# OpenGene/gencore

Hardware: AMD Instinct MI355X
Metric: consensus read-pairs/sec (whole node) + clustering HBM GB/s vs roofline (higher is better)
Workload: dtype u8

## Files before the change

gencore_amd/csrc/engine.hip:

```cpp
#include <hip/hip_runtime.h>
#include <hip/hip_ext.h>
#include <cstdio>
#include <cstdlib>
#include <algorithm>
#include <cstring>
#include <ctime>
#include <string>
#include <vector>

#include "gce_entry.h"
#include "gce_kernels.hpp"
#include "gce_params.hpp"
#include "gce_pair2.hpp"
#include "gce_vote.hpp"
#include "gce_deep.hpp"
#include "gce_output.hpp"
#include "gce_depth.hpp"
#include "gce_inflate.hpp"
#include "gce_deflate.hpp"

namespace {

static thread_local double t_alloc_s = 0.0; static thread_local long t_alloc_n = 0; static thread_local size_t t_alloc_bytes = 0;
static inline double mono_s() { struct timespec ts; clock_gettime(CLOCK_MONOTONIC, &ts); return (double)ts.tv_sec + 1e-9 * (double)ts.tv_nsec; }
// ... 22 lines not shown
struct ScopedBuf : DevBuf { ~ScopedBuf() { release(); } };
template <class T> inline hipError_t ensure_as(DevBuf &d, T *&dst, size_t bytes) { const hipError_t r = d.ensure(bytes); dst = d.as<T>(); return r; }

enum { EV_START = 0, EV_CLUSTER, EV_CSR, EV_DESCRIBE, EV_PAIRING, EV_SCORE, EV_CONSENSUS, EV_FINISH, EV_OUTPUT, EV_COUNT };

}

#include "gce_devstream.hpp"

struct HostRaw {
    uint8_t *p = nullptr; size_t n = 0, cap = 0;
    ~HostRaw() { free(p); }
    void resize(size_t k) { if (k > cap) { free(p); p = (uint8_t *)malloc(k ? k : 1); cap = p ? k : 0; } n = p ? k : 0; }
    uint8_t *data() { return p; }
    size_t size() const { return n; }
    bool empty() const { return n == 0; }
};

struct gce_engine {
    gce_params prm{};
    bool vote_off_logged = false;
    std::vector<uint32_t> target_len;
    std::string err;
    hipStream_t stream = nullptr;
    hipEvent_t ev[EV_COUNT]{};
    std::vector<DevBuf> ref_buf; std::vector<const uint8_t *> ref_ptr; std::vector<int64_t> ref_len, ref_win; bool have_win = false;
    DevBuf d_ref_ptr, d_ref_len, d_ref_win, d_target_len, d_target_cum;
    std::vector<const uint8_t *> up_ref_ptr; std::vector<int64_t> up_ref_len, up_win; std::vector<uint32_t> up_tl; const void *up_dev[5]{}; bool up_valid = false;
    std::vector<gce_core> h_core; std::vector<uint64_t> h_qoff, h_coff, h_soff, h_loff, h_mioff;
    std::vector<char> h_qname, h_mi; std::vector<uint32_t> h_cigar; std::vector<uint8_t> h_seq, h_qual, h_nmt; std::vector<int32_t> h_nm; std::vector<uint64_t> h_tick;
    std::vector<int32_t> h_ev_tid, h_ev_pos;
    bool have_mi = false, have_tick = false, have_events = false, host_mode = false, device_mode = false, processed = false;
    bool reserved = false; hipStream_t up_stream = nullptr; std::vector<hipEvent_t> up_events;
    hipStream_t aux_stream = nullptr; hipEvent_t aux_ev[4]{};
    size_t rs_n = 0, rs_q = 0, rs_c = 0, rs_s = 0, rs_l = 0, st_n = 0, st_q = 0, st_c = 0, st_s = 0, st_l = 0, st_m = 0; bool dev_concat = false;
    gce_batch dev_batch{};
    DevBuf b_core, b_qoff, b_qname, b_coff, b_cigar, b_soff, b_seq, b_loff, b_qual, b_nm, b_nmt, b_mioff, b_mi, b_tick;
    DevBuf uinfo, rdesc, spatch, slot, score, out_flag, orec, out_index, nmx;
    DevBuf o_src, o_kind, o_qsrc, o_nm, o_fr, o_rr, o_mate, o_soff, o_qoff, o_seq, o_qual, o_key, o_rec, o_ksoff, o_kqoff, o_krow, o_rank64, o_part3, ref_ascii;
    int64_t n_out = 0; size_t out_seq_bytes = 0, out_qual_bytes = 0; int dev_error = 0; uint32_t dev_error_read = 0;
    DevBuf lrec, lout, bhdr, blk_base, ev_tid, ev_pos, ev_read, table, toff;
    DevBuf raw, rw_tmp, rw_ncig, rw_nmpos, rw_rsize, rw_roff, rw_body; RecIdx rw;
    size_t raw_n = 0; bool raw_mode = false; int64_t raw_records = 0; uint64_t raw_body_bytes = 0;
    int64_t idx_ctr[4] = {0, 0, 0, 0};
    DevBuf z_comp, z_dir, z_err; size_t z_n = 0; std::vector<InfDir> z_members;
    DevBuf zo_slots, zo_sizes, zo_off, zo_out; uint64_t zo_bytes = 0;
    DevBuf sf_text; uint64_t sf_bytes = 0; int64_t raw_body_nrec = -1;
    std::vector<gce_engine *> mirrors;
    DevBuf sh_tickall, sh_shard, sh_flag, sh_sel, sh_core, sh_qoff, sh_coff, sh_soff, sh_loff, sh_nm, sh_nmt, sh_mioff, sh_tick, sh_roff, sh_nmpos, sh_keys, sh_stage; int64_t shard_n = -1;
    bool shard_cut_done = false;
    bool tab_clean = false; const void *tab_clean_ptr = nullptr; size_t tab_clean_cap = 0;
    DevBuf cl_ikey, cl_start, cl_n, cl_npairs, cl_ngroups, cl_gbase, cl_nresult, cl_hasumi, cl_tier;
    DevBuf members, sorted, pl, pr, pu, pg, gpl, gpr, grp_begin, grp_n, gl_cluster, g_begin, g_np;
    DevBuf slow_args, deep_list, k64, slow_list, left_list, pf_flag, pf_list, pq_flag, pq_list, p16_flag, p16_list, pd_slab, gen_flag, gen_list, score_list, gw, vlive, vb_start, rp_left, rp_right, rp_merge, rp_rmerge, rp_umi, rp_umilen, rp_state, rp_supp, rp_nm, rp_qsl, rp_qsr, scan_part, si;
    StreamInfo h_si{};
    void *si_pin = nullptr, *si_pin_dev = nullptr; unsigned long long si_seq = 0;
    gce_timing timing{};
    int64_t n = 0, n_pre = 0;
    DevBuf dp_binoff, dp_regoff, dp_rs, dp_re, dp_pmax, dp_sorted, dp_depth, dp_bed, dp_where;
    std::vector<int64_t> h_binoff, h_depth_pre, h_depth_post, h_bed_pre, h_bed_post; int64_t payload_words = 0;
    std::vector<uint8_t> r_kind; HostRaw r_seq, r_qual; std::vector<uint32_t> r_src, r_qsrc, r_mate; std::vector<int32_t> r_nm; std::vector<int16_t> r_fr, r_rr;
    std::vector<uint64_t> r_soff, r_qoff;
};

static int fail(gce_engine *e, int code, const std::string &msg) { if (e) e->err = msg; return code; }
#define HIPCHK(call) do { hipError_t _e = (call); if (_e != hipSuccess) return fail(e, _e == hipErrorOutOfMemory ? GCE_ERR_OOM : GCE_ERR_HIP, std::string(#call) + ": " + hipGetErrorString(_e)); } while (0)

extern "C" {

int gce_abi_version(void) { return GCE_ABI_VERSION; }

void gce_params_default(gce_params *p) {
    memset(p, 0, sizeof *p);
    p->abi_version = GCE_ABI_VERSION;
    p->proper_umi_diff_threshold = 1; p->unproper_umi_diff_threshold = 0; p->duplex_mismatch_threshold = 2;
    p->cluster_size_req = 1; p->base_score_req = 6; p->high_quality = 30; p->moderate_quality = 20; p->low_quality = 15;
    p->score_high = 8; p->score_moderate = 6; p->score_low = 4; p->score_bad = 2;
    p->skip_low_complexity_cluster_threshold = 1000; p->flush_period = 10000; p->score_percent_req = 0.8;
}

void gce_detect_umi_prefix(const char *q, char out[32]) {
    memset(out, 0, 32);
    if (strstr(q, "umi_")) strcpy(out, "umi");
    else if (strstr(q, "UMI_")) strcpy(out, "UMI");
}

const char *gce_status_message(int s) {
    switch (s) {
    case GCE_OK: return "ok";
    case GCE_ERR_INVALID: return "invalid argument or call order";
    case GCE_ERR_NO_DEVICE: return "no HIP device available (this engine has no CPU fallback)";
    case GCE_ERR_HIP: return "HIP runtime error";
    case GCE_ERR_OOM: return "out of device memory";
    case GCE_ERR_UNSORTED: return "ERROR: the input is unsorted. Please sort the input first.";
    case GCE_ERR_UMI_MISMATCH: return "The UMI of a read pair should be identical";
    case GCE_ERR_NM_MISSING: return "NM tag missing on a consensus template whose mismatch count changed";
    case GCE_ERR_UMI_PARSE: return "UMI parse: substr start beyond the end of the read name";
    case GCE_ERR_QNAME_SHORT: return "copyQName ERROR: desitination qname is shorter";
    case GCE_ERR_REF_WINDOW: return "reference window: a clustered read lies outside the bases staged for its contig";
    default: return "unknown status";
    }
}

const char *gce_last_error(const gce_engine *e) { return e ? e->err.c_str() : "null engine"; }

int gce_create(const gce_params *params, gce_engine **out) {
    if (!params || !out || params->abi_version != GCE_ABI_VERSION) return GCE_ERR_INVALID;
    if (params->proper_umi_diff_threshold < 0 || params->unproper_umi_diff_threshold < 0 || params->flush_period < 0) return GCE_ERR_INVALID;
    int ndev = 0;
    if (hipGetDeviceCount(&ndev) != hipSuccess || ndev <= 0 || params->device >= ndev) return GCE_ERR_NO_DEVICE;
    gce_engine *e = new gce_engine();
    e->prm = *params;
    if (e->prm.flush_period == 0) e->prm.flush_period = 10000;
    if (params->n_targets > 0 && params->target_len) e->target_len.assign(params->target_len, params->target_len + params->n_targets);
    e->prm.target_len = nullptr;
    if (hipSetDevice(params->device) != hipSuccess || hipStreamCreate(&e->stream) != hipSuccess) { delete e; return GCE_ERR_HIP; }
    for (auto &v : e->ev) (void)hipEventCreate(&v);
    *out = e;
    return GCE_OK;
}

void gce_destroy(gce_engine *e) {
    if (!e) return;
    (void)hipSetDevice(e->prm.device);
    (void)hipStreamSynchronize(e->stream);
    DevBuf *all[] = {&e->d_ref_ptr, &e->d_ref_len, &e->d_ref_win, &e->d_target_len, &e->d_target_cum, &e->b_core, &e->b_qoff, &e->b_qname, &e->b_coff, &e->b_cigar, &e->b_soff,
                     &e->b_seq, &e->b_loff, &e->b_qual, &e->b_nm, &e->b_nmt, &e->b_mioff, &e->b_mi, &e->b_tick, &e->uinfo, &e->rdesc, &e->spatch,
                     &e->slot, &e->score, &e->out_flag, &e->orec, &e->out_index, &e->nmx, &e->o_src, &e->o_kind, &e->o_qsrc, &e->o_nm, &e->o_fr, &e->o_rr, &e->o_mate,
                     &e->o_key, &e->o_rec, &e->o_ksoff, &e->o_kqoff, &e->o_krow, &e->o_rank64, &e->o_part3, &e->o_soff, &e->o_qoff, &e->o_seq, &e->o_qual, &e->ref_ascii, &e->lrec, &e->lout, &e->bhdr,
                     &e->blk_base, &e->ev_tid, &e->ev_pos, &e->ev_read, &e->table, &e->toff, &e->cl_ikey, &e->cl_start, &e->cl_n,
                     &e->cl_npairs, &e->cl_ngroups, &e->cl_gbase, &e->cl_nresult, &e->cl_hasumi, &e->cl_tier, &e->members, &e->sorted, &e->pl, &e->pr, &e->pu,
                     &e->pg, &e->gpl, &e->gpr, &e->grp_begin, &e->grp_n, &e->gl_cluster, &e->g_begin, &e->g_np, &e->deep_list, &e->k64, &e->slow_list, &e->pf_flag, &e->pf_list, &e->pq_flag, &e->pq_list, &e->left_list, &e->slow_args, &e->pd_slab, &e->gen_flag, &e->gen_list, &e->score_list, &e->gw, &e->vlive, &e->vb_start, &e->rp_left, &e->rp_right, &e->rp_merge, &e->rp_rmerge,
                     &e->rp_umi, &e->rp_umilen, &e->rp_state, &e->rp_supp, &e->rp_nm, &e->rp_qsl, &e->rp_qsr, &e->scan_part, &e->si};
    for (auto *b : all) b->release();
    for (DevBuf *b : {&e->z_comp, &e->z_dir, &e->z_err, &e->raw, &e->rw_tmp, &e->rw_ncig, &e->rw_nmpos, &e->rw_rsize, &e->rw_roff, &e->rw_body, &e->sf_text}) b->release();
    e->rw.release();
    for (DevBuf *b : {&e->zo_slots, &e->zo_sizes, &e->zo_off, &e->zo_out, &e->p16_flag, &e->p16_list}) b->release();
    for (DevBuf *b : {&e->sh_tickall, &e->sh_shard, &e->sh_flag, &e->sh_sel, &e->sh_core, &e->sh_qoff, &e->sh_coff, &e->sh_soff, &e->sh_loff, &e->sh_nm, &e->sh_nmt, &e->sh_mioff, &e->sh_tick, &e->sh_roff, &e->sh_nmpos, &e->sh_keys, &e->sh_stage}) b->release();
    for (DevBuf *b : {&e->dp_binoff, &e->dp_regoff, &e->dp_rs, &e->dp_re, &e->dp_pmax, &e->dp_sorted, &e->dp_depth, &e->dp_bed, &e->dp_where}) b->release();
    for (auto ev : e->up_events) (void)hipEventDestroy(ev);
    if (e->up_stream) { (void)hipStreamSynchronize(e->up_stream); (void)hipStreamDestroy(e->up_stream); }
    if (e->aux_stream) { (void)hipStreamSynchronize(e->aux_stream); (void)hipStreamDestroy(e->aux_stream); }
    for (auto &v : e->aux_ev) if (v) (void)hipEventDestroy(v);
    for (auto &b : e->ref_buf) b.release();
    for (auto &v : e->ev) if (v) (void)hipEventDestroy(v);
    if (e->stream) (void)hipStreamDestroy(e->stream);
    if (e->si_pin) (void)hipHostFree(e->si_pin);
    delete e;
}

void gce_pack_reference(const char *bases, int64_t n, uint8_t *out) {
    memset(out, 0, (size_t)((n + 1) / 2));
    for (int64_t i = 0; i < n; i++) {
        uint8_t code;
        switch (bases[i]) { case 'A': code = 1; break; case 'T': code = 2; break; case 'C': code = 3; break; case 'G': code = 4; break; default: code = 0; }
        out[i >> 1] |= (i & 1) ? (uint8_t)(code << 4) : code;
    }
}

int gce_set_reference(gce_engine *e, int32_t tid, const uint8_t *nibbles, int64_t n_bases) {
    if (!e || tid < 0 || n_bases < 0) return GCE_ERR_INVALID;
    (void)hipSetDevice(e->prm.device);
    if ((size_t)tid >= e->ref_buf.size()) { e->ref_buf.resize(tid + 1); e->ref_ptr.resize(tid + 1, nullptr); e->ref_len.resize(tid + 1, 0); }
    if (!nibbles) { e->ref_ptr[tid] = nullptr; e->ref_len[tid] = 0; return GCE_OK; }
    size_t bytes = (size_t)((n_bases + 1) / 2);
    HIPCHK(e->ref_buf[tid].ensure(bytes + 16));
    hipPointerAttribute_t attr; bool is_dev = hipPointerGetAttributes(&attr, nibbles) == hipSuccess && attr.type == hipMemoryTypeDevice;
    (void)hipGetLastError();
    HIPCHK(hipMemcpyAsync(e->ref_buf[tid].p, nibbles, bytes, is_dev ? hipMemcpyDeviceToDevice : hipMemcpyHostToDevice, e->stream));
    HIPCHK(hipStreamSynchronize(e->stream));
    e->ref_ptr[tid] = e->ref_buf[tid].as<uint8_t>(); e->ref_len[tid] = n_bases;
    if (2 * (size_t)tid + 1 < e->ref_win.size()) e->ref_win[2 * tid] = e->ref_win[2 * tid + 1] = 0;
    return GCE_OK;
}

int gce_set_reference_ascii(gce_engine *e, int32_t tid, const char *bases, int64_t n_bases) {
    if (!e || tid < 0 || n_bases < 0 || (!bases && n_bases > 0)) return GCE_ERR_INVALID;
    (void)hipSetDevice(e->prm.device);
    if ((size_t)tid >= e->ref_buf.size()) { e->ref_buf.resize(tid + 1); e->ref_ptr.resize(tid + 1, nullptr); e->ref_len.resize(tid + 1, 0); }
    const size_t bytes = (size_t)((n_bases + 1) / 2);
    HIPCHK(e->ref_buf[tid].ensure(bytes + 16));
    HIPCHK(e->ref_ascii.ensure((size_t)n_bases + 16));
    hipPointerAttribute_t attr; const bool is_dev = hipPointerGetAttributes(&attr, bases) == hipSuccess && attr.type == hipMemoryTypeDevice;
    (void)hipGetLastError();
    if (n_bases) {
        HIPCHK(hipMemcpyAsync(e->ref_ascii.p, bases, (size_t)n_bases, is_dev ? hipMemcpyDeviceToDevice : hipMemcpyHostToDevice, e->stream));
        const unsigned grid = (unsigned)std::min<uint64_t>((bytes + 255) / 256, 65535u * 4u);
        hipLaunchKernelGGL(k_pack_reference, dim3(grid), dim3(256), 0, e->stream, (const char *)e->ref_ascii.p, n_bases, e->ref_buf[tid].as<uint8_t>());
    }
    HIPCHK(hipStreamSynchronize(e->stream));
// ... 511 lines not shown
        CANARY("EV_CLUSTER");
        if (N > 0) {
            if (!e->have_tick) {
                hipLaunchKernelGGL(k_blk_scan, dim3(1), dim3(1024), 0, s, w, p);
                hipLaunchKernelGGL(k_events, dim3(cdiv(max_events, EV_T / 64)), dim3(EV_T), 0, s, b, p, w);
            }
            const unsigned nb4 = cdiv(n_sblk, 4);
            hipLaunchKernelGGL(k_leaders, dim3(nb4), dim3(256), 0, s, b, p, w);
            hipLaunchKernelGGL(k_num_reduce, dim3(nb4), dim3(256), 0, s, w, p.nw_cb);
            hipLaunchKernelGGL(k_scan_partials, dim3(1), dim3(1024), 0, s, w.scan_part, (uint64_t)nb4, &w.si->n_clusters, (unsigned long long *)nullptr);
            hipLaunchKernelGGL(k_num_apply, dim3(nb4), dim3(256), 0, s, w);
            LAUNCH_EV(k_scatter, dim3((unsigned)n_sblk), dim3(SB_T), s, e->ev[EV_CSR], N, w);
        } else HIPCHK(hipEventRecord(e->ev[EV_CSR], s));
        CANARY("EV_CSR");
        return GCE_OK;
    }

    int describe() {
        int rc;
        unsigned long long si_seq1 = 0;
        if ((rc = read_si_begin(e, &si_seq1)) != GCE_OK) return rc;
        if (N > 0) {
#ifndef GCE_DESCRIBE_BLOCKS
#define GCE_DESCRIBE_BLOCKS 32768
#endif
            const int64_t n_tiles = (N + 255) / 256;
            int tpb = (int)((n_tiles + GCE_DESCRIBE_BLOCKS - 1) / GCE_DESCRIBE_BLOCKS); if (tpb < 1) tpb = 1;
            LAUNCH_EV(k_describe, dim3(cdiv(n_tiles, tpb)), dim3(256), s, e->ev[EV_DESCRIBE], b, p, w, tpb);
        } else HIPCHK(hipEventRecord(e->ev[EV_DESCRIBE], s));
        CANARY("EV_DESCRIBE");
        if ((rc = read_si_end(e, si_seq1)) != GCE_OK) return rc;
        HIPCHK(hipGetLastError());
        e->tab_clean = true;
        C = (uint32_t)e->h_si.n_clusters;
        const size_t c1 = C ? C : 1;
        TAKE(cl_npairs, w.cl_npairs, c1 * 4); TAKE(cl_ngroups, w.cl_ngroups, c1 * 4); TAKE(cl_gbase, w.cl_gbase, c1 * 4); TAKE(cl_nresult, w.cl_nresult, c1 * 4);
        TAKE(cl_hasumi, w.cl_hasumi, c1); TAKE(cl_tier, w.cl_tier, c1);
        return GCE_OK;
    }

    void compact_flags(uint8_t *flag, uint32_t *list, unsigned long long *count) {
        const unsigned nbc = cdiv(C, SCAN_TILE);
        hipLaunchKernelGGL(k_flag_reduce, dim3(nbc), dim3(256), 0, s, (const uint8_t *)flag, (uint64_t)C, w.scan_part);
        hipLaunchKernelGGL(k_scan_partials, dim3(1), dim3(1024), 0, s, w.scan_part, (uint64_t)nbc, count, (unsigned long long *)nullptr);
        hipLaunchKernelGGL(k_flag_apply, dim3(nbc), dim3(256), 0, s, (const uint8_t *)flag, (uint64_t)C, (const uint64_t *)w.scan_part, list);
    }

    int pair_clusters() {
        if (!(C > 0 && e->dev_error == 0)) { HIPCHK(hipEventRecord(e->ev[EV_PAIRING], s)); return GCE_OK; }
        int rc;
        const size_t c1 = C;
        TAKE(left_list, w.left_list, c1 * 4 + 64);
        TAKE(pf_flag, w.pf_flag, c1 + 64); TAKE(pf_list, w.pf_list, c1 * 4); TAKE(pq_flag, w.pq_flag, c1 + 64); TAKE(pq_list, w.pq_list, c1 * 4); TAKE(p16_flag, w.p16_flag, c1 + 64); TAKE(p16_list, w.p16_list, c1 * 4);
        const bool pair_classes = (double)N > 10.0 * (double)C;
        if (!pair_classes) fill_many(s, {FillSeg{e->pf_flag.p, c1, 0u, 0u}, FillSeg{e->pq_flag.p, c1, 0u, 0u}});
        const unsigned nbc = cdiv(C, SCAN_TILE);
#ifdef PS_STOP
        return time_pairing_sub_and_stop();
#endif
        HIPCHK(e->pd_slab.ensure(PD_BIG_BLOCKS * PD_SLAB));
        if (pair_classes) {
            hipLaunchKernelGGL(k_pair_class_reduce, dim3(nbc), dim3(256), 0, s, (const uint32_t *)w.cl_n, C, w.scan_part);
            hipLaunchKernelGGL(k_scan_partials, dim3(1), dim3(1024), 0, s, w.scan_part, (uint64_t)nbc, &w.si->n_p16_items, &w.si->n_pq_items);
            hipLaunchKernelGGL(k_pair_class_apply, dim3(nbc), dim3(256), 0, s, (const uint32_t *)w.cl_n, C, (const uint64_t *)w.scan_part, w.p16_list, w.pq_list, w.pf_list, w.si);
            static const bool tiers_aux = getenv("GCE_NO_AUX_STREAM") == nullptr;
            hipStream_t s2 = s;
            if (tiers_aux) {
                if ((rc = aux_ready(e)) != GCE_OK) return rc;
                s2 = e->aux_stream;
                HIPCHK(hipEventRecord(e->aux_ev[0], s));
                HIPCHK(hipStreamWaitEvent(s2, e->aux_ev[0], 0));
            }
            hipLaunchKernelGGL(k_pairing_fast, dim3(2048), dim3(256), 0, s2, b, p, w, C, (const uint32_t *)w.pf_list);
            hipLaunchKernelGGL(k_pairing_deep<false>, dim3(256), dim3(PD_T), 0, s2, b, p, w, (uint8_t *)nullptr);
            if (tiers_aux) HIPCHK(hipEventRecord(e->aux_ev[1], s2));
            hipLaunchKernelGGL(k_pairing_sub<16>, dim3(cdiv(C, 4 * WAVES_PER_BLOCK)), dim3(256), 0, s, b, p, w, C, (const uint32_t *)w.p16_list, (const unsigned long long *)&w.si->n_p16_items, w.pq_flag, 1);
            hipLaunchKernelGGL(k_pairing_sub<32>, dim3(cdiv(C, 2 * WAVES_PER_BLOCK)), dim3(256), 0, s, b, p, w, C, (const uint32_t *)w.pq_list, (const unsigned long long *)&w.si->n_pq_items, w.pf_flag, 1);
            if (tiers_aux) HIPCHK(hipStreamWaitEvent(s, e->aux_ev[1], 0));
        } else {
            hipLaunchKernelGGL(k_pairing_sub<16>, dim3(cdiv(C, 4 * WAVES_PER_BLOCK)), dim3(256), 0, s, b, p, w, C, (const uint32_t *)nullptr, (const unsigned long long *)nullptr, w.pq_flag, 0);
            compact_flags(w.pq_flag, w.pq_list, &w.si->n_pq_items);
            hipLaunchKernelGGL(k_pairing_sub<32>, dim3(cdiv(C, 2 * WAVES_PER_BLOCK)), dim3(256), 0, s, b, p, w, C, (const uint32_t *)w.pq_list, (const unsigned long long *)&w.si->n_pq_items, w.pf_flag, 0);
            compact_flags(w.pf_flag, w.pf_list, &w.si->n_pf_items);
            hipLaunchKernelGGL(k_pairing_fast, dim3(2048), dim3(256), 0, s, b, p, w, C, (const uint32_t *)w.pf_list);
            hipLaunchKernelGGL(k_pairing_deep<false>, dim3(256), dim3(PD_T), 0, s, b, p, w, (uint8_t *)nullptr);
        }
        hipLaunchKernelGGL(k_pairing_deep<true>, dim3(PD_BIG_BLOCKS), dim3(PD_T), 0, s, b, p, w, e->pd_slab.as<uint8_t>());
        hipLaunchKernelGGL(k_pairing_slow<0>, dim3(1024), dim3(256), 0, s, b, p, w);
        hipLaunchKernelGGL(k_pairing_slow<1>, dim3(1024, 16), dim3(256), 0, s, b, p, w);
        hipLaunchKernelGGL(k_pairing_slow<2>, dim3(1024), dim3(256), 0, s, b, p, w);
        hipLaunchKernelGGL(k_scan_reduce, dim3(nbc), dim3(256), 0, s, (const uint32_t *)w.cl_ngroups, (uint64_t)C, w.scan_part);
        hipLaunchKernelGGL(k_scan_partials, dim3(1), dim3(1024), 0, s, w.scan_part, (uint64_t)nbc, &w.si->n_pairs , &w.si->n_groups);
        hipLaunchKernelGGL(k_u32_apply, dim3(nbc), dim3(256), 0, s, (const uint32_t *)w.cl_ngroups, w.cl_gbase, (uint64_t)C, (const uint64_t *)w.scan_part);
        TAKE(gl_cluster, w.gl_cluster, n1 * 4); TAKE(g_begin, w.g_begin, n1 * 4); TAKE(g_np, w.g_np, n1 * 4); TAKE(gw, w.gw, n1 * 8); TAKE(vlive, w.vlive, n1 * 16);
        const size_t vb_cap = ((VB_MINW + 3) * n1) / VB_W + 8;
        TAKE(vb_start, w.vb_start, vb_cap * 4);
        HIPCHK(hipMemsetAsync(e->vb_start.p, 0xFF, vb_cap * 4, s));
        hipLaunchKernelGGL(k_group_fill, dim3(cdiv(C, 256)), dim3(256), 0, s, p, w, C, (uint32_t)VB_W, (uint32_t)VB_MINW);
        hipLaunchKernelGGL(k_u64_reduce, dim3(nblk_N), dim3(256), 0, s, (const uint64_t *)w.gw, (const unsigned long long *)&w.si->n_groups, w.scan_part);
        hipLaunchKernelGGL(k_u64_partials, dim3(1), dim3(1024), 0, s, w.scan_part, (const unsigned long long *)&w.si->n_groups, &w.si->vote_weight, &w.si->n_live);
        LAUNCH_EV(k_vote_batches, dim3(nblk_N), dim3(256), s, e->ev[EV_PAIRING], w, (const unsigned long long *)&w.si->n_groups, (const uint64_t *)w.scan_part);
        CANARY("EV_PAIRING");
        if ((rc = read_si(e)) != GCE_OK) return rc;
        HIPCHK(hipGetLastError());
        si_behind_describe = true;
        NG = (uint32_t)e->h_si.n_groups;
        return GCE_OK;
    }

    int consensus() {
        int rc;
        const size_t g1 = NG ? NG : 1;
        TAKE(gen_list, w.gen_list, g1 * 8); TAKE(gen_flag, w.gen_flag, g1 * 2 + 64);
        TAKE(score_list, w.score_list, n1 * 4 + 64);
        TAKE(rp_left, w.rp_left, g1 * 4); TAKE(rp_right, w.rp_right, g1 * 4); TAKE(rp_merge, w.rp_merge, g1 * 4); TAKE(rp_rmerge, w.rp_rmerge, g1 * 4); TAKE(rp_umi, w.rp_umi, g1 * 8);
        TAKE(rp_umilen, w.rp_umilen, g1 * 2); TAKE(rp_state, w.rp_state, g1); TAKE(rp_supp, w.rp_supp, g1 * 4); TAKE(rp_nm, w.rp_nm, g1 * 8); TAKE(rp_qsl, w.rp_qsl, g1 * 4); TAKE(rp_qsr, w.rp_qsr, g1 * 4);
        if (NG > 0 && e->dev_error == 0) {
            {
                SlowArgs sa; sa.b = b; sa.p = p; sa.w = w;
                HIPCHK(e->slow_args.ensure(sizeof sa));
                HIPCHK(hipMemcpyAsync(e->slow_args.p, &sa, sizeof sa, hipMemcpyHostToDevice, s));
            }
            fill_many(s, {FillSeg{e->gen_flag.p, g1 * 2, 0u, 0u},
                          FillSeg{e->rp_nm.p, g1 * 8, 0xFFu, 0u},
                          FillSeg{e->rp_left.p, g1 * 4, 0xFFu, 0u}, FillSeg{e->rp_right.p, g1 * 4, 0xFFu, 0u}});
            const uint32_t n_live = (uint32_t)e->h_si.n_live;
#ifdef VB_XCD
            const unsigned nbatch = (((unsigned)(e->h_si.vote_weight / VB_W) + 1u) + 7u) & ~7u;
#else
            const unsigned nbatch = (unsigned)(e->h_si.vote_weight / VB_W) + 1u;
#endif
#ifdef VB_STOP
            return time_vote_and_stop(nbatch, n_live);
#endif
            LAUNCH_EV(k_vote, dim3(nbatch), dim3(VB_T), s, e->ev[EV_SCORE], b, p, w, n_live);
            CANARY("EV_SCORE");
            const bool deep_stream = ((double)N > 48.0 * (double)NG || getenv("GCE_FORCE_AUX_STREAM")) && !getenv("GCE_NO_AUX_STREAM");
            const unsigned cf_cap = deep_stream ? 32768u : 4096u, sc2_cap = deep_stream ? 16384u : 2048u;
            const unsigned cf_grid = std::min<unsigned>(cdiv(2ull * NG, WAVES_PER_BLOCK), cf_cap);
            const unsigned sc2_grid = std::min<unsigned>(cdiv(N, 2 * WAVES_PER_BLOCK * 64), sc2_cap);
            if (deep_stream) {
                if ((rc = aux_ready(e)) != GCE_OK) return rc;
                HIPCHK(hipEventRecord(e->aux_ev[0], s));
                HIPCHK(hipStreamWaitEvent(e->aux_stream, e->aux_ev[0], 0));
                hipLaunchKernelGGL(k_score2, dim3(sc2_grid), dim3(256), 0, e->aux_stream, b, p, w);
                HIPCHK(hipEventRecord(e->aux_ev[1], e->aux_stream));
                hipLaunchKernelGGL(k_deep_prepare, dim3(1024), dim3(256), 0, s, b, p, w);
                HIPCHK(hipStreamWaitEvent(s, e->aux_ev[1], 0));
                hipLaunchKernelGGL(k_consensus_fast, dim3(cf_grid), dim3(256), 0, s, b, p, w);
            } else {
                hipLaunchKernelGGL(k_score2, dim3(sc2_grid), dim3(256), 0, s, b, p, w);
                hipLaunchKernelGGL(k_deep_prepare, dim3(1024), dim3(256), 0, s, b, p, w);
                hipLaunchKernelGGL(k_consensus_fast, dim3(cf_grid), dim3(256), 0, s, b, p, w);
            }
            hipLaunchKernelGGL(k_vote_deep, dim3(1024), dim3(DV_T), 0, s, b, p, w);
            LAUNCH_EV(k_consensus_slow, dim3(512), dim3(256), s, e->ev[EV_CONSENSUS], (const SlowArgs *)e->slow_args.p);
            CANARY("EV_CONSENSUS");
            hipLaunchKernelGGL(k_group_tail, dim3(cdiv(NG, 256)), dim3(256), 0, s, b, p, w, NG);
            if (!p.disable_duplex) {
// ... 367 lines not shown
```

gencore_amd/csrc/gce_device.hpp:

```cpp
#pragma once
#include <hip/hip_runtime.h>
#include <stdint.h>
#include "../../include/gencore_amd.h"

#define GCE_WAVE 64
#define NONE32 0xFFFFFFFFu
#define EMPTY64 0xFFFFFFFFFFFFFFFFull

enum : uint32_t { THR_PROPER = 0, THR_UNPROPER = 1, THR_NEVER = 2, THR_RAW = 3 };
enum : uint8_t { TIER_NEVER = 0, TIER_SUB16 = 1, TIER_SUB32 = 2, TIER_FAST = 3, TIER_DEEP_LDS = 4, TIER_DEEP_DEVICE = 5, TIER_GENERIC = 6 };
enum : uint8_t { CLS_DROP = 0, CLS_CLUSTERED = 1, CLS_BYPASS = 2 };

struct DevBatch {
    int64_t n;
    const gce_core *core;
    const uint64_t *qname_off; const char *qname;
    const uint64_t *cigar_off; const uint32_t *cigar;
    const uint64_t *seq_off;   uint8_t *seq;
    const uint64_t *qual_off;  uint8_t *qual;
    const int32_t *nm; const uint8_t *nm_type;
    const uint64_t *mi_off; const char *mi;
    const uint64_t *tick;
};

struct DevParams {
    int32_t proper_thr, unproper_thr, duplex_mismatch_thr, cluster_size_req, base_score_req;
    int32_t high_q, moderate_q, low_q;
    int32_t s_high, s_moderate, s_low, s_bad;
    int32_t skip_low_complexity_thr, duplex_only, disable_duplex, period;
    int32_t score_bias, score_max;
    uint32_t q2s_lut;
    uint32_t thr_low4, thr_mod4, thr_high4;
    int32_t q2s_swar_ok;
    double score_percent_req;
    char prefix[32];
    int32_t prefix_len;
    int32_t n_targets;
    const uint32_t *target_len;
    const uint64_t *target_cum;
    int32_t key_bt, key_bl;
    int32_t nw_ok, nw_cb, nw_bd;
    int32_t vote_ok, vote_accept_by_qual, s_min_lb;
    int64_t tick_offset;
    int64_t tick_epoch0; int32_t tick_rem0;
    int32_t trailing_flush;
    int32_t n_ref;
    const uint8_t *const *ref_data;
    const int64_t *ref_len;
    const int64_t *ref_win;
};

#define GCE_PRE_SLOTS 64
struct StreamInfo {
    unsigned long long n_clustered;
    unsigned int first_unmapped;
    unsigned long long err_key;
    int n_events;
    int n_events_a;
    unsigned int n_slow;
    unsigned long long prof[32];
    unsigned int n_deep;
    unsigned long long hand_on;
    unsigned int n_slow_pair;
    unsigned int n_slow_pair2;
    unsigned int pair_next, pair_next2;
    unsigned int prep_next, deep_next;
    int lq_min, lq_max;
    unsigned long long n_clusters, n_groups, n_pairs, n_out;
    unsigned long long n_pairs_total;
    unsigned long long vote_weight;
    unsigned long long n_live;
    unsigned long long n_leaders;
    unsigned long long out_units;
    unsigned long long n_pf_items;
    unsigned long long n_pq_items;
    unsigned long long n_p16_items;
    unsigned long long vote_rounds2;
    unsigned long long vote_rounds2_unaligned;
    unsigned int n_raw;
    unsigned int cs_fast, cs_prep, cs_deep, cs_slow;
    long long pre[GCE_STATS_WORDS];
    long long post[GCE_STATS_WORDS];
    long long post_slot[GCE_PRE_SLOTS][8];
    long long pre_slot[GCE_PRE_SLOTS][8];
};

__device__ __forceinline__ void raise_error(StreamInfo *si, int code, uint32_t read) {
    atomicMin(&si->err_key, ((unsigned long long)read << 8) | (unsigned long long)((-code) & 0xFF));
}

__device__ __forceinline__ int lane_id() { return threadIdx.x & 63; }

__device__ __forceinline__ int cig_op(uint32_t w) { return (int)(w & 0xF); }
__device__ __forceinline__ int cig_len(uint32_t w) { return (int)(w >> 4); }
__device__ __forceinline__ int consumes_query(int op) { return (0x193 >> op) & 1; }
__device__ __forceinline__ int consumes_ref(int op) { return (0x18D >> op) & 1; }

struct __attribute__((aligned(16))) ReadDescP {
    uint32_t so_lo, qo_lo;
    uint32_t c0;
    uint32_t pos_fl;
    uint16_t lq, mo, ml, nc;
    int32_t tid;
    uint32_t hi;
};
static_assert(sizeof(ReadDescP) == 32, "ReadDescP must stay 32 bytes");
struct ReadDesc {
    uint64_t so, qo;
    uint32_t c0;
    int32_t pos, lq, isize;
    int32_t mo, ml;
    int32_t tid;
    uint16_t nc, lastm;
    int32_t rlen;
};
#define RLEN_WALK (-0x40000000)
__device__ __forceinline__ void store_desc(ReadDescP *base, uint64_t i, uint64_t so, uint64_t qo, uint32_t c0, int32_t pos, bool isize_nz, int lq, int mo, int ml, int nc, int32_t tid, uint32_t last_op) {
    union { ReadDescP d; uint4 q[2]; } u;
    u.d.so_lo = (uint32_t)so; u.d.qo_lo = (uint32_t)qo; const uint32_t lastm = cig_op(last_op) == 0 ? min((uint32_t)cig_len(last_op), 65535u) : 0u;
    u.d.hi = ((uint32_t)(so >> 32) & 0xFFu) | ((uint32_t)(qo >> 32) & 0xFFu) << 8 | lastm << 16;
    u.d.c0 = c0; u.d.pos_fl = (uint32_t)pos | (isize_nz ? 0x80000000u : 0u);
    u.d.lq = (uint16_t)lq; u.d.mo = (uint16_t)mo; u.d.ml = (uint16_t)ml; u.d.nc = (uint16_t)nc; u.d.tid = tid;
    uint4 *dst = reinterpret_cast<uint4 *>(base + i); dst[0] = u.q[0]; dst[1] = u.q[1];
}
__device__ __forceinline__ ReadDesc load_desc(const ReadDescP *base, uint32_t i) {
    union { ReadDescP d; uint4 q[2]; } u;
    const uint4 *src = reinterpret_cast<const uint4 *>(base + i);
    u.q[0] = src[0]; u.q[1] = src[1];
    ReadDesc r;
// ... 335 lines not shown
```

gencore_amd/csrc/gce_kernels.hpp:

```cpp
#pragma once
#include "gce_device.hpp"

#define CHUNK 256
#define WAVES_PER_BLOCK 4

struct __attribute__((aligned(16))) OutRec { uint32_t qname_src, mate; int16_t nm_new, fr, rr; uint16_t pad; };
static_assert(sizeof(OutRec) == 16, "OutRec must stay 16 bytes");

struct Work {
    uint64_t *uinfo;
    ReadDescP *rdesc;
    uint32_t *spatch;
    uint32_t *slot;
    int8_t *score;
    uint8_t *out_flag; OutRec *orec;
    uint32_t *nmx;
    uint32_t *out_index;
    struct LeadRec *lrec; struct LeadOut *lout;
    struct BlkHdr *bhdr; uint32_t *blk_base; int64_t n_sblk;
    int32_t *ev_tid, *ev_pos; uint32_t *ev_read; int max_events;
    struct TabEntry *tab; uint32_t *toff; uint64_t tsize; double tinv;
    uint32_t *cl_ikey, *cl_start, *cl_n, *cl_npairs, *cl_ngroups, *cl_gbase, *cl_nresult; uint8_t *cl_hasumi;
    uint8_t *cl_tier;
    uint32_t *members, *sorted, *pl, *pr, *pu, *pg, *gpl, *gpr, *grp_begin, *grp_n;
    uint64_t *k64;
    uint32_t *gl_cluster, *g_begin, *g_np;
    uint64_t *gw; uint4 *vlive; uint32_t *vb_start;
    uint32_t *slow_list;
    uint8_t *pf_flag; uint32_t *pf_list;
    uint8_t *pq_flag; uint32_t *pq_list;
    uint32_t *left_list;
    uint8_t *p16_flag; uint32_t *p16_list;
    void *deep_list;
    uint8_t *gen_flag; uint32_t *gen_list;
    uint32_t *score_list;
    uint32_t *rp_left, *rp_right, *rp_merge, *rp_rmerge; const char **rp_umi; uint16_t *rp_umilen; uint8_t *rp_state; int32_t *rp_supp;
    int32_t *rp_nm;
    uint32_t *rp_qsl, *rp_qsr;
    uint64_t *scan_part;
    StreamInfo *si;
};

#define UINFO_MAXLEN 32767
__device__ __forceinline__ uint64_t uinfo_pack(uint64_t off, bool from_mi, int l_qname, int len) {
    return (off & 0xFFFFFFFFFFull) | ((uint64_t)(from_mi ? 1 : 0) << 40) | ((uint64_t)(l_qname & 0xFF) << 41) | ((uint64_t)(len & 0x7FFF) << 49);
}
__device__ __forceinline__ const char *uinfo_ptr(const DevBatch &b, uint64_t v) { return (((v >> 40) & 1ull) ? b.mi : b.qname) + (v & 0xFFFFFFFFFFull); }
__device__ __forceinline__ int uinfo_len(uint64_t v) { return (int)(v >> 49); }
__device__ __forceinline__ bool uinfo_hm(uint64_t v) { return ((v >> 40) & 1ull) != 0; }
__device__ __forceinline__ int uinfo_lqname_pad(uint64_t v) { return ((int)((v >> 41) & 0xFFu) + 3) & ~3; }
__device__ __forceinline__ const char *d_umi_ptr(const DevBatch &b, const Work &w, uint64_t i) { return uinfo_ptr(b, w.uinfo[i]); }
__device__ __forceinline__ int d_umi_len(const Work &w, uint64_t i) { return uinfo_len(w.uinfo[i]); }
__device__ __forceinline__ bool d_umi_hm(const Work &w, uint64_t i) { return uinfo_hm(w.uinfo[i]); }
__device__ __forceinline__ int d_lqname(const Work &w, uint64_t i) { return (int)((w.uinfo[i] >> 41) & 0xFFu); }

enum : uint8_t { RP_PENDING = 0, RP_OUT_SSCS = 1, RP_OUT_DCS = 2, RP_DROPPED = 3, RP_CONSUMED = 4 };
#define NM_DEFER (-0x40000000)
#define NM_IS_DEFERRED(v) ((v) < -0x20000000)

#define WAVE_SYNC() do { __builtin_amdgcn_fence(__ATOMIC_SEQ_CST, "workgroup"); __builtin_amdgcn_wave_barrier(); } while (0)

__device__ __forceinline__ int rl32(int v, int l) { return __builtin_amdgcn_readlane(v, l); }
__device__ __forceinline__ uint64_t rl64(uint64_t v, int l) {
    uint32_t lo = (uint32_t)__builtin_amdgcn_readlane((int)(uint32_t)v, l), hi = (uint32_t)__builtin_amdgcn_readlane((int)(uint32_t)(v >> 32), l);
    return ((uint64_t)hi << 32) | lo;
}

__device__ __forceinline__ long long wave_sum64(long long v) {
    for (int o = 32; o > 0; o >>= 1) v += __shfl_xor(v, o);
    return v;
}

#include "gce_cluster.hpp"

__device__ __forceinline__ const char *d_qname(const DevBatch &b, uint32_t r) { return b.qname + b.qname_off[r]; }

typedef uint64_t u64_unaligned __attribute__((aligned(1)));
typedef uint32_t u32_unaligned __attribute__((aligned(1)));
__device__ __forceinline__ uint64_t d_bswap64(uint64_t x) { return __builtin_bswap64(x); }
template <int NW>
__device__ __forceinline__ void load_be_words(const char *s, int len, uint64_t (&wd)[NW]) {
#pragma unroll
    for (int k = 0; k < NW; k++) {
        uint64_t v = 0;
        int rem = len - 8 * k;
// ... 1779 lines not shown
```

gencore_amd/csrc/gce_pair2.hpp:

```cpp
#pragma once

template <int SUB> __device__ __forceinline__ int sub_max(int v) {
    v = row_max16(v);
    if (SUB == 32) { const int t = __shfl_xor(v, 16); v = t > v ? t : v; }
    return v;
}
template <int SUB> __device__ __forceinline__ uint32_t sub_ballot(bool pr, int hb) {
    const unsigned long long m = __ballot(pr);
    return (uint32_t)(m >> hb) & (SUB == 32 ? 0xFFFFFFFFu : ((1u << (SUB & 31)) - 1u));
}
__device__ __forceinline__ uint64_t shfl64(uint64_t v, int src) { return (uint64_t)__shfl((long long)v, src); }

__device__ __forceinline__ int pair_class(uint32_t n) { return n <= 16u ? 0 : (n <= 32u ? 1 : 2); }
__global__ __launch_bounds__(256) void k_pair_class_reduce(const uint32_t *cl_n, uint32_t n_clusters, uint64_t *part) {
    __shared__ uint64_t s[4];
    const uint64_t base = (uint64_t)blockIdx.x * SCAN_TILE;
    uint64_t v = 0;
    for (int k = 0; k < SCAN_TILE / 256; k++) {
        const uint64_t i = base + k * 256 + threadIdx.x;
        if (i < n_clusters) { const int c = pair_class(cl_n[i]); v += c == 0 ? (1ull << 32) : (c == 1 ? 1ull : 0ull); }
    }
    v = (uint64_t)wave_sum64((long long)v);
    if (lane_id() == 0) s[threadIdx.x >> 6] = v;
    __syncthreads();
    if (threadIdx.x == 0) part[blockIdx.x] = s[0] + s[1] + s[2] + s[3];
}
__global__ __launch_bounds__(256) void k_pair_class_apply(const uint32_t *cl_n, uint32_t n_clusters, const uint64_t *part, uint32_t *l16, uint32_t *l32, uint32_t *l64, StreamInfo *si) {
    __shared__ uint32_t s_w[4][2];
    __shared__ uint32_t s_c0, s_c1;
    const int lane = lane_id(), wv = threadIdx.x >> 6;
    const uint64_t base = (uint64_t)blockIdx.x * SCAN_TILE;
    if (threadIdx.x == 0) { s_c0 = (uint32_t)(part[blockIdx.x] >> 32); s_c1 = (uint32_t)part[blockIdx.x]; }
    if (blockIdx.x == 0 && threadIdx.x == 0) si->n_pf_items = (unsigned long long)n_clusters - si->n_p16_items - si->n_pq_items;
    __syncthreads();
    for (int k = 0; k < SCAN_TILE / 256; k++) {
        const uint64_t i = base + k * 256 + threadIdx.x;
        const int c = i < n_clusters ? pair_class(cl_n[i]) : -1;
        const unsigned long long m0 = __ballot(c == 0), m1 = __ballot(c == 1);
        if (lane == 0) { s_w[wv][0] = (uint32_t)__popcll(m0); s_w[wv][1] = (uint32_t)__popcll(m1); }
        __syncthreads();
        uint32_t o0 = s_c0, o1 = s_c1, t0 = 0, t1 = 0;
        for (int q = 0; q < 4; q++) { if (q < wv) { o0 += s_w[q][0]; o1 += s_w[q][1]; } t0 += s_w[q][0]; t1 += s_w[q][1]; }
        const uint32_t r0 = o0 + (uint32_t)lanes_below(m0), r1 = o1 + (uint32_t)lanes_below(m1);
        if (c == 0) l16[r0] = (uint32_t)i;
        else if (c == 1) l32[r1] = (uint32_t)i;
        else if (c == 2) l64[(uint32_t)i - r0 - r1] = (uint32_t)i;
        __syncthreads();
        if (threadIdx.x == 0) { s_c0 += t0; s_c1 += t1; }
        __syncthreads();
    }
}
#ifdef PS_STOP
#define PS_TICK(k, live_) do { if ((k) >= PS_STOP) { if ((uint32_t)(live_) == 0xDEADBEEFu) flag_out[0] = 1; return; } } while (0)
#else
#define PS_TICK(k, live_) do { } while (0)
#endif
template <int SUB>
__global__ __launch_bounds__(256) void k_pairing_sub(DevBatch b, DevParams p, Work w, uint32_t n_clusters, const uint32_t *list, const unsigned long long *list_n, uint8_t *flag_out, int direct) {
    constexpr int PER = 64 / SUB;
    const int lane = lane_id(), hl = lane & (SUB - 1), hb = lane & ~(SUB - 1);
    const uint32_t idx = (blockIdx.x * WAVES_PER_BLOCK + (threadIdx.x >> 6)) * PER + (uint32_t)(lane / SUB);
    const uint32_t total = list ? (uint32_t)*list_n : n_clusters;
    if ((blockIdx.x * WAVES_PER_BLOCK + (threadIdx.x >> 6)) * PER >= total) return;
    bool live = idx < total;
    const uint32_t c = live ? (list ? list[idx] : idx) : 0u;
    uint32_t start = 0, n = 0; int thr = 0;
    if (live) {
        start = w.cl_start[c]; n = w.cl_n[c];
        const uint32_t mode = d_thr_mode(w.cl_ikey[c], w.si, p);
        if (mode >= THR_NEVER) { if (hl == 0) { w.cl_npairs[c] = 0; w.cl_ngroups[c] = 0; w.cl_hasumi[c] = 0; w.cl_tier[c] = TIER_NEVER; } live = false; }
        thr = mode == THR_PROPER ? p.proper_thr : p.unproper_thr;
    }
    uint32_t my = NONE32; int nl = 0; const char *nm = nullptr; int ul = 0;
    const char *up = nullptr;
    if (live && n <= (uint32_t)SUB && hl < (int)n) {
        my = w.members[start + hl];
        const uint64_t ui_ = w.uinfo[my];
        nl = (int)((ui_ >> 41) & 0xFFu) - 1;
        nm = d_qname(b, my);
        ul = uinfo_len(ui_);
        up = uinfo_ptr(b, ui_);
    }
    const uint32_t toolong = sub_ballot<SUB>(nl > 64 || ul > 24, hb);
    if (live && (n > (uint32_t)SUB || toolong)) {
        if (hl == 0) { if (direct) w.left_list[atomicAdd(&w.si->n_slow_pair2, 1u)] = c; else flag_out[c] = 1; }
        live = false;
    }
    if (!__any(live)) return;
    PS_TICK(0, my ^ (uint32_t)nl ^ (uint32_t)ul ^ (uint32_t)(uintptr_t)nm ^ (uint32_t)(uintptr_t)up);
    const bool act = live && hl < (int)n;
    const int nwords = (wave_max_u(act ? nl : 0) + 7) >> 3;
    uint64_t nw[8];
#pragma unroll
    for (int k = 0; k < 8; k++) {
        uint64_t v = 0;
        if (k < nwords) {
            const int rem = (act ? nl : 0) - 8 * k;
            if (rem > 0) { v = *(const u64_unaligned *)(nm + 8 * k); if (rem < 8) v &= (1ull << (8 * rem)) - 1ull; v = d_bswap64(v); }
        }
        nw[k] = v;
    }
    uint64_t ruw[3];
// ... 197 lines not shown
```

Measured before the change: 1.909 billion.

## Add one-thread-per-cluster pairing path for clusters of at most two reads

Adds a fourth pair class for clusters with one or two reads. The class is compacted into its own list by extending the reduce, scan and apply kernels, and a new k_pairing_tiny kernel handles each such cluster in a single thread, comparing names and UMIs directly. Previously these clusters were processed by the 16-lane sub-wave pairing kernel, which wastes most lanes on tiny clusters. The cost is a second scan segment, more divergent per-thread logic, and a fallback to the slow path on hash collisions or long names. An optional env var prints class counts.

```diff
diff --git a/gencore_amd/csrc/engine.hip b/gencore_amd/csrc/engine.hip
--- a/gencore_amd/csrc/engine.hip
+++ b/gencore_amd/csrc/engine.hip
@@ -98,7 +98,7 @@
     bool tab_clean = false; const void *tab_clean_ptr = nullptr; size_t tab_clean_cap = 0;
     DevBuf cl_ikey, cl_start, cl_n, cl_npairs, cl_ngroups, cl_gbase, cl_nresult, cl_hasumi, cl_tier;
     DevBuf members, sorted, pl, pr, pu, pg, gpl, gpr, grp_begin, grp_n, gl_cluster, g_begin, g_np;
-    DevBuf slow_args, deep_list, k64, slow_list, left_list, pf_flag, pf_list, pq_flag, pq_list, p16_flag, p16_list, pd_slab, gen_flag, gen_list, score_list, gw, vlive, vb_start, rp_left, rp_right, rp_merge, rp_rmerge, rp_umi, rp_umilen, rp_state, rp_supp, rp_nm, rp_qsl, rp_qsr, scan_part, si;
+    DevBuf slow_args, deep_list, k64, slow_list, left_list, pf_flag, pf_list, pq_flag, pq_list, p16_flag, p16_list, pt_list, pd_slab, gen_flag, gen_list, score_list, gw, vlive, vb_start, rp_left, rp_right, rp_merge, rp_rmerge, rp_umi, rp_umilen, rp_state, rp_supp, rp_nm, rp_qsl, rp_qsr, scan_part, si;
     StreamInfo h_si{};
     void *si_pin = nullptr, *si_pin_dev = nullptr; unsigned long long si_seq = 0;
     gce_timing timing{};
@@ -181,7 +181,7 @@
     for (auto *b : all) b->release();
     for (DevBuf *b : {&e->z_comp, &e->z_dir, &e->z_err, &e->raw, &e->rw_tmp, &e->rw_ncig, &e->rw_nmpos, &e->rw_rsize, &e->rw_roff, &e->rw_body, &e->sf_text}) b->release();
     e->rw.release();
-    for (DevBuf *b : {&e->zo_slots, &e->zo_sizes, &e->zo_off, &e->zo_out, &e->p16_flag, &e->p16_list}) b->release();
+    for (DevBuf *b : {&e->zo_slots, &e->zo_sizes, &e->zo_off, &e->zo_out, &e->p16_flag, &e->p16_list, &e->pt_list}) b->release();
     for (DevBuf *b : {&e->sh_tickall, &e->sh_shard, &e->sh_flag, &e->sh_sel, &e->sh_core, &e->sh_qoff, &e->sh_coff, &e->sh_soff, &e->sh_loff, &e->sh_nm, &e->sh_nmt, &e->sh_mioff, &e->sh_tick, &e->sh_roff, &e->sh_nmpos, &e->sh_keys, &e->sh_stage}) b->release();
     for (DevBuf *b : {&e->dp_binoff, &e->dp_regoff, &e->dp_rs, &e->dp_re, &e->dp_pmax, &e->dp_sorted, &e->dp_depth, &e->dp_bed, &e->dp_where}) b->release();
     for (auto ev : e->up_events) (void)hipEventDestroy(ev);
@@ -799,6 +799,7 @@
         const size_t c1 = C;
         TAKE(left_list, w.left_list, c1 * 4 + 64);
         TAKE(pf_flag, w.pf_flag, c1 + 64); TAKE(pf_list, w.pf_list, c1 * 4); TAKE(pq_flag, w.pq_flag, c1 + 64); TAKE(pq_list, w.pq_list, c1 * 4); TAKE(p16_flag, w.p16_flag, c1 + 64); TAKE(p16_list, w.p16_list, c1 * 4);
+        TAKE(pt_list, w.pt_list, c1 * 4);
         const bool pair_classes = (double)N > 10.0 * (double)C;
         if (!pair_classes) fill_many(s, {FillSeg{e->pf_flag.p, c1, 0u, 0u}, FillSeg{e->pq_flag.p, c1, 0u, 0u}});
         const unsigned nbc = cdiv(C, SCAN_TILE);
@@ -808,8 +809,8 @@
         HIPCHK(e->pd_slab.ensure(PD_BIG_BLOCKS * PD_SLAB));
         if (pair_classes) {
             hipLaunchKernelGGL(k_pair_class_reduce, dim3(nbc), dim3(256), 0, s, (const uint32_t *)w.cl_n, C, w.scan_part);
-            hipLaunchKernelGGL(k_scan_partials, dim3(1), dim3(1024), 0, s, w.scan_part, (uint64_t)nbc, &w.si->n_p16_items, &w.si->n_pq_items);
-            hipLaunchKernelGGL(k_pair_class_apply, dim3(nbc), dim3(256), 0, s, (const uint32_t *)w.cl_n, C, (const uint64_t *)w.scan_part, w.p16_list, w.pq_list, w.pf_list, w.si);
+            hipLaunchKernelGGL(k_scan_partials, dim3(1), dim3(1024), 0, s, w.scan_part, (uint64_t)2 * nbc, &w.si->n_pt_items, &w.si->n_pq_items);
+            hipLaunchKernelGGL(k_pair_class_apply, dim3(nbc), dim3(256), 0, s, (const uint32_t *)w.cl_n, C, (const uint64_t *)w.scan_part, w.p16_list, w.pq_list, w.pf_list, w.pt_list, w.si);
             static const bool tiers_aux = getenv("GCE_NO_AUX_STREAM") == nullptr;
             hipStream_t s2 = s;
             if (tiers_aux) {
@@ -818,6 +819,7 @@
                 HIPCHK(hipEventRecord(e->aux_ev[0], s));
                 HIPCHK(hipStreamWaitEvent(s2, e->aux_ev[0], 0));
             }
+            hipLaunchKernelGGL(k_pairing_tiny, dim3(std::min<unsigned>(cdiv(C, 256), 1024u)), dim3(256), 0, s2, b, p, w, (const uint32_t *)w.pt_list, (const unsigned long long *)&w.si->n_pt_items);
             hipLaunchKernelGGL(k_pairing_fast, dim3(2048), dim3(256), 0, s2, b, p, w, C, (const uint32_t *)w.pf_list);
             hipLaunchKernelGGL(k_pairing_deep<false>, dim3(256), dim3(PD_T), 0, s2, b, p, w, (uint8_t *)nullptr);
             if (tiers_aux) HIPCHK(hipEventRecord(e->aux_ev[1], s2));
@@ -852,6 +854,10 @@
         HIPCHK(hipGetLastError());
         si_behind_describe = true;
         NG = (uint32_t)e->h_si.n_groups;
+        static const bool class_counts = getenv("GCE_PAIR_CLASS_COUNTS") != nullptr;
+        if (class_counts && pair_classes)
+            fprintf(stderr, "pair classes: %u clusters, %lld reads; <= 2 reads %llu, 3..16 %llu, 17..32 %llu, more %llu\n", C, (long long)N, e->h_si.n_pt_items, e->h_si.n_p16_items,
+                    e->h_si.n_pq_items, e->h_si.n_pf_items);
         return GCE_OK;
     }
 
diff --git a/gencore_amd/csrc/gce_device.hpp b/gencore_amd/csrc/gce_device.hpp
--- a/gencore_amd/csrc/gce_device.hpp
+++ b/gencore_amd/csrc/gce_device.hpp
@@ -75,6 +75,7 @@
     unsigned long long n_pf_items;
     unsigned long long n_pq_items;
     unsigned long long n_p16_items;
+    unsigned long long n_pt_items;
     unsigned long long vote_rounds2;
     unsigned long long vote_rounds2_unaligned;
     unsigned int n_raw;
diff --git a/gencore_amd/csrc/gce_kernels.hpp b/gencore_amd/csrc/gce_kernels.hpp
--- a/gencore_amd/csrc/gce_kernels.hpp
+++ b/gencore_amd/csrc/gce_kernels.hpp
@@ -31,6 +31,7 @@
     uint8_t *pq_flag; uint32_t *pq_list;
     uint32_t *left_list;
     uint8_t *p16_flag; uint32_t *p16_list;
+    uint32_t *pt_list;
     void *deep_list;
     uint8_t *gen_flag; uint32_t *gen_list;
     uint32_t *score_list;
diff --git a/gencore_amd/csrc/gce_pair2.hpp b/gencore_amd/csrc/gce_pair2.hpp
--- a/gencore_amd/csrc/gce_pair2.hpp
+++ b/gencore_amd/csrc/gce_pair2.hpp
@@ -11,43 +11,124 @@
 }
 __device__ __forceinline__ uint64_t shfl64(uint64_t v, int src) { return (uint64_t)__shfl((long long)v, src); }
 
-__device__ __forceinline__ int pair_class(uint32_t n) { return n <= 16u ? 0 : (n <= 32u ? 1 : 2); }
+__device__ __forceinline__ int pair_class(uint32_t n) { return n <= 2u ? 3 : (n <= 16u ? 0 : (n <= 32u ? 1 : 2)); }
 __global__ __launch_bounds__(256) void k_pair_class_reduce(const uint32_t *cl_n, uint32_t n_clusters, uint64_t *part) {
-    __shared__ uint64_t s[4];
+    __shared__ uint64_t s[4][2];
     const uint64_t base = (uint64_t)blockIdx.x * SCAN_TILE;
-    uint64_t v = 0;
+    uint64_t v = 0, t = 0;
     for (int k = 0; k < SCAN_TILE / 256; k++) {
         const uint64_t i = base + k * 256 + threadIdx.x;
-        if (i < n_clusters) { const int c = pair_class(cl_n[i]); v += c == 0 ? (1ull << 32) : (c == 1 ? 1ull : 0ull); }
-    }
-    v = (uint64_t)wave_sum64((long long)v);
-    if (lane_id() == 0) s[threadIdx.x >> 6] = v;
+        if (i < n_clusters) { const int c = pair_class(cl_n[i]); v += c == 0 ? (1ull << 32) : (c == 1 ? 1ull : 0ull); t += c == 3 ? (1ull << 32) : 0ull; }
+    }
+    v = (uint64_t)wave_sum64((long long)v); t = (uint64_t)wave_sum64((long long)t);
+    if (lane_id() == 0) { s[threadIdx.x >> 6][0] = v; s[threadIdx.x >> 6][1] = t; }
     __syncthreads();
-    if (threadIdx.x == 0) part[blockIdx.x] = s[0] + s[1] + s[2] + s[3];
-}
-__global__ __launch_bounds__(256) void k_pair_class_apply(const uint32_t *cl_n, uint32_t n_clusters, const uint64_t *part, uint32_t *l16, uint32_t *l32, uint32_t *l64, StreamInfo *si) {
-    __shared__ uint32_t s_w[4][2];
-    __shared__ uint32_t s_c0, s_c1;
+    if (threadIdx.x == 0) { part[blockIdx.x] = s[0][0] + s[1][0] + s[2][0] + s[3][0]; part[gridDim.x + blockIdx.x] = s[0][1] + s[1][1] + s[2][1] + s[3][1]; }
+}
+__global__ __launch_bounds__(256) void k_pair_class_apply(const uint32_t *cl_n, uint32_t n_clusters, const uint64_t *part, uint32_t *l16, uint32_t *l32, uint32_t *l64, uint32_t *lt, StreamInfo *si) {
+    __shared__ uint32_t s_w[4][3];
+    __shared__ uint32_t s_c0, s_c1, s_c3;
     const int lane = lane_id(), wv = threadIdx.x >> 6;
     const uint64_t base = (uint64_t)blockIdx.x * SCAN_TILE;
-    if (threadIdx.x == 0) { s_c0 = (uint32_t)(part[blockIdx.x] >> 32); s_c1 = (uint32_t)part[blockIdx.x]; }
-    if (blockIdx.x == 0 && threadIdx.x == 0) si->n_pf_items = (unsigned long long)n_clusters - si->n_p16_items - si->n_pq_items;
+    if (threadIdx.x == 0) { s_c0 = (uint32_t)(part[blockIdx.x] >> 32); s_c1 = (uint32_t)part[blockIdx.x]; s_c3 = (uint32_t)((part[gridDim.x + blockIdx.x] - part[gridDim.x]) >> 32); }
+    if (blockIdx.x == 0 && threadIdx.x == 0) {
+        const unsigned long long n16 = part[gridDim.x] >> 32, nt = si->n_pt_items - n16;
+        si->n_p16_items = n16; si->n_pt_items = nt; si->n_pf_items = (unsigned long long)n_clusters - n16 - nt - si->n_pq_items;
+    }
     __syncthreads();
     for (int k = 0; k < SCAN_TILE / 256; k++) {
         const uint64_t i = base + k * 256 + threadIdx.x;
         const int c = i < n_clusters ? pair_class(cl_n[i]) : -1;
-        const unsigned long long m0 = __ballot(c == 0), m1 = __ballot(c == 1);
-        if (lane == 0) { s_w[wv][0] = (uint32_t)__popcll(m0); s_w[wv][1] = (uint32_t)__popcll(m1); }
+        const unsigned long long m0 = __ballot(c == 0), m1 = __ballot(c == 1), m3 = __ballot(c == 3);
+        if (lane == 0) { s_w[wv][0] = (uint32_t)__popcll(m0); s_w[wv][1] = (uint32_t)__popcll(m1); s_w[wv][2] = (uint32_t)__popcll(m3); }
         __syncthreads();
-        uint32_t o0 = s_c0, o1 = s_c1, t0 = 0, t1 = 0;
-        for (int q = 0; q < 4; q++) { if (q < wv) { o0 += s_w[q][0]; o1 += s_w[q][1]; } t0 += s_w[q][0]; t1 += s_w[q][1]; }
-        const uint32_t r0 = o0 + (uint32_t)lanes_below(m0), r1 = o1 + (uint32_t)lanes_below(m1);
+        uint32_t o0 = s_c0, o1 = s_c1, o3 = s_c3, t0 = 0, t1 = 0, t3 = 0;
+        for (int q = 0; q < 4; q++) { if (q < wv) { o0 += s_w[q][0]; o1 += s_w[q][1]; o3 += s_w[q][2]; } t0 += s_w[q][0]; t1 += s_w[q][1]; t3 += s_w[q][2]; }
+        const uint32_t r0 = o0 + (uint32_t)lanes_below(m0), r1 = o1 + (uint32_t)lanes_below(m1), r3 = o3 + (uint32_t)lanes_below(m3);
         if (c == 0) l16[r0] = (uint32_t)i;
         else if (c == 1) l32[r1] = (uint32_t)i;
-        else if (c == 2) l64[(uint32_t)i - r0 - r1] = (uint32_t)i;
+        else if (c == 3) lt[r3] = (uint32_t)i;
+        else if (c == 2) l64[(uint32_t)i - r0 - r1 - r3] = (uint32_t)i;
         __syncthreads();
-        if (threadIdx.x == 0) { s_c0 += t0; s_c1 += t1; }
+        if (threadIdx.x == 0) { s_c0 += t0; s_c1 += t1; s_c3 += t3; }
         __syncthreads();
+    }
+}
+__device__ __forceinline__ uint64_t tiny_name_word(const char *nm, int nl, int k) {
+    const int rem = nl - 8 * k;
+    if (rem <= 0) return 0ull;
+    uint64_t v = *(const u64_unaligned *)(nm + 8 * k);
+    if (rem < 8) v &= (1ull << (8 * rem)) - 1ull;
+    return d_bswap64(v);
+}
+__device__ __forceinline__ uint32_t tiny_h32_step(uint32_t h, uint64_t v) {
+    const uint32_t lo = (uint32_t)v, hi = (uint32_t)(v >> 32);
+    h = (__builtin_rotateleft32(h, 5) ^ lo) + hi;
+    return __builtin_rotateleft32(h, 11) ^ (hi + 0x7F4A7C15u);
+}
+__global__ __launch_bounds__(256) void k_pairing_tiny(DevBatch b, DevParams p, Work w, const uint32_t *list, const unsigned long long *list_n) {
+    const uint32_t total = (uint32_t)*list_n, stride = gridDim.x * blockDim.x;
+    for (uint32_t idx = blockIdx.x * blockDim.x + threadIdx.x; idx < total; idx += stride) {
+        const uint32_t c = list[idx];
+        const uint32_t start = w.cl_start[c], n = w.cl_n[c];
+        const uint32_t mode = d_thr_mode(w.cl_ikey[c], w.si, p);
+        if (mode >= THR_NEVER) { w.cl_npairs[c] = 0; w.cl_ngroups[c] = 0; w.cl_hasumi[c] = 0; w.cl_tier[c] = TIER_NEVER; continue; }
+        const int thr = mode == THR_PROPER ? p.proper_thr : p.unproper_thr;
+        const uint32_t m0 = w.members[start], m1 = n > 1u ? w.members[start + 1] : NONE32;
+        const uint32_t ra = m1 < m0 ? m1 : m0, rb = m1 < m0 ? m0 : m1;
+        const uint64_t ua = w.uinfo[ra], ub = n > 1u ? w.uinfo[rb] : 0ull;
+        const int nla = (int)((ua >> 41) & 0xFFu) - 1, nlb = n > 1u ? (int)((ub >> 41) & 0xFFu) - 1 : 0;
+        const int ula = uinfo_len(ua), ulb = n > 1u ? uinfo_len(ub) : 0;
+        if (nla > 64 || nlb > 64 || ula > 24 || ulb > 24) { w.left_list[atomicAdd(&w.si->n_slow_pair2, 1u)] = c; continue; }
+        uint64_t wa[3], wb[3];
+        load_be_words<3>(uinfo_ptr(b, ua), ula, wa);
+        load_be_words<3>(n > 1u ? uinfo_ptr(b, ub) : nullptr, ulb, wb);
+        uint32_t npairs = 1, ngroups = 1; bool any_umi;
+        if (n <= 1u) {
+            any_umi = ula > 0;
+            w.gpl[start] = ra; w.gpr[start] = NONE32;
+            w.grp_begin[start] = start; w.grp_n[start] = 1;
+        } else {
+            const char *na = d_qname(b, ra), *nb = d_qname(b, rb);
+            const int nwords = ((nla > nlb ? nla : nlb) + 7) >> 3;
+            uint32_t ha = 0x9E3779B9u, hb = 0x9E3779B9u; int cmp = 0;
+            for (int k = 0; k < nwords; k++) {
+                const uint64_t x = tiny_name_word(na, nla, k), y = tiny_name_word(nb, nlb, k);
+                ha = tiny_h32_step(ha, x); hb = tiny_h32_step(hb, y);
+                if (cmp == 0) cmp = x < y ? -1 : (x > y ? 1 : 0);
+            }
+            ha ^= ha >> 15; hb ^= hb >> 15;
+            if (cmp == 0) {
+                if (ula != 0 && !(ula == ulb && wa[0] == wb[0] && wa[1] == wb[1] && wa[2] == wb[2])) raise_error(w.si, GCE_ERR_UMI_MISMATCH, rb);
+                any_umi = ulb > 0;
+                w.gpl[start] = ra; w.gpr[start] = rb;
+                w.grp_begin[start] = start; w.grp_n[start] = 1;
+            } else {
+                if (ha == hb) { w.left_list[atomicAdd(&w.si->n_slow_pair2, 1u)] = c; continue; }
+                npairs = 2;
+                any_umi = ula > 0 || ulb > 0;
+                const bool swp = cmp > 0;
+                const uint32_t p0 = swp ? rb : ra, p1 = swp ? ra : rb;
+                bool split = false, top1 = false;
+                if (any_umi) {
+                    const bool lt_ba = wb[0] != wa[0] ? wb[0] < wa[0] : (wb[1] != wa[1] ? wb[1] < wa[1] : (wb[2] != wa[2] ? wb[2] < wa[2] : ulb < ula));
+                    const bool lt_ab = wa[0] != wb[0] ? wa[0] < wb[0] : (wa[1] != wb[1] ? wa[1] < wb[1] : (wa[2] != wb[2] ? wa[2] < wb[2] : ula < ulb));
+                    top1 = swp ? lt_ab : lt_ba;
+                    split = popc_nonzero_bytes(wa[0] ^ wb[0]) + popc_nonzero_bytes(wa[1] ^ wb[1]) + popc_nonzero_bytes(wa[2] ^ wb[2]) > thr;
+                }
+                if (split) {
+                    ngroups = 2;
+                    w.gpl[start] = top1 ? p1 : p0; w.gpl[start + 1] = top1 ? p0 : p1;
+                    w.grp_begin[start] = start; w.grp_n[start] = 1; w.grp_begin[start + 1] = start + 1; w.grp_n[start + 1] = 1;
+                } else {
+                    w.gpl[start] = p0; w.gpl[start + 1] = p1;
+                    w.grp_begin[start] = start; w.grp_n[start] = 2;
+                }
+                w.gpr[start] = NONE32; w.gpr[start + 1] = NONE32;
+            }
+        }
+        const bool cross = d_key(b.core[m0], p).right < 0;
+        w.cl_npairs[c] = npairs; w.cl_ngroups[c] = ngroups; w.cl_hasumi[c] = (uint8_t)((any_umi ? 1 : 0) | (cross ? 2 : 0)); w.cl_tier[c] = TIER_SUB16;
     }
 }
 #ifdef PS_STOP
```

Result: no change. 1.916 billion (median of 2 runs) (+0.4%).
